# kwea123/ngp_pl

Measured on NVIDIA H100. Metric: train_rays_per_sec, higher is better.
Workload: dtype f16

## Files before the change

ngp_pl_b200/csrc/network.cu:

```cuda
#include "common.cuh"
#include "hashgrid.cuh"
#include "mlp.cuh"
#include "wgmma.cuh"
#include "../../include/ngp_b200.h"
#include <math.h>

extern "C" int ngp_abi_version(void) { return NGP_ABI_VERSION; }

unsigned long long g_ngp_launch_count = 0;
extern "C" unsigned long long ngp_launch_count(void) { return __atomic_load_n(&g_ngp_launch_count, __ATOMIC_RELAXED); }

unsigned long long* g_ngp_trace = nullptr;
__global__ void k_trace_stamp(unsigned long long* buf, int id) { trace_mark(buf, id); }
void ngp_trace_stamp(int id, cudaStream_t st) { k_trace_stamp<<<1, 1, 0, st>>>(g_ngp_trace, id); }
extern "C" int ngp_trace_set(void* buf) {
    g_ngp_trace = (unsigned long long*)buf;
    return 0;
}

extern "C" uint32_t ngp_grid_meta(int n_levels, int log2_hashmap_size, int base_resolution, float per_level_scale,
                                  NgpGridMeta* out) {
    if (!out || n_levels < 1 || n_levels > NGP_MAX_LEVELS || log2_hashmap_size < 3 || log2_hashmap_size > 28 ||
        base_resolution < 1 || !(per_level_scale >= 1.0f))
        return 0;
    const float log2_b = log2f(per_level_scale);
    uint64_t offset = 0;
    out->n_levels = n_levels;
    out->hashed_mask = 0;
    for (int l = 0; l < NGP_MAX_LEVELS; ++l) {
        out->offset[l] = 0; out->res[l] = 0; out->scale[l] = 0.f;
    }
    for (int l = 0; l < n_levels; ++l) {
        const float scale = exp2f((float)l * log2_b) * (float)base_resolution - 1.0f;
        const uint32_t res = (uint32_t)ceilf(scale) + 1u;
        const uint64_t dense = (uint64_t)res * res * res;
        uint64_t entries = (dense + 7u) / 8u * 8u;
        const uint64_t cap = 1ull << log2_hashmap_size;
        if (entries > cap) entries = cap;
        if (dense > entries) out->hashed_mask |= (1u << l);
        out->offset[l] = (uint32_t)offset;
        out->res[l] = res;
        out->scale[l] = scale;
        offset += entries;
        if (offset > 0xffffffffull) return 0;
    }
    for (int l = n_levels; l <= NGP_MAX_LEVELS; ++l) out->offset[l] = (uint32_t)offset;
    return (uint32_t)offset;
}

__global__ void k_cast_params(const float* __restrict__ src, __half* __restrict__ dst, int64_t n) {
    const int64_t i = (blockIdx.x * (int64_t)blockDim.x + threadIdx.x) * 4;
    if (i + 3 < n && ((((uintptr_t)src) & 15) == 0) && ((((uintptr_t)dst) & 7) == 0)) {
        const float4 v = *reinterpret_cast<const float4*>(src + i);
        uint2 o;
        o.x = pack_half2(v.x, v.y);
        o.y = pack_half2(v.z, v.w);
        *reinterpret_cast<uint2*>(dst + i) = o;
    } else {
        for (int64_t k = i; k < n && k < i + 4; ++k) dst[k] = __float2half_rn(src[k]);
    }
}
extern "C" int ngp_cast_params(const float* src, uint16_t* dst_half, int64_t n, void* stream) {
    if (n < 0) return NGP_EINVAL;
    if (n == 0) return 0;
    k_cast_params<<<ngp_div_up((n + 3) / 4, 256), 256, 0, (cudaStream_t)stream>>>(src, (__half*)dst_half, n);
    NGP_CHECK_LAUNCH();
    return 0;
}

#define NGP_SCHED_EAGER 1024
#define NGP_SCHED_GRAPH 1024
__device__ int g_sched[NGP_SCHED_EAGER + NGP_SCHED_GRAPH][2];
static int* sched_slot(cudaStream_t st) {
    static int* bases[64] = {nullptr};
    static unsigned eager_seq[64] = {0}, graph_seq[64] = {0};
    int dev = 0;
    if (cudaGetDevice(&dev) != cudaSuccess || dev < 0 || dev >= 64) return nullptr;
    int* base = __atomic_load_n(&bases[dev], __ATOMIC_ACQUIRE);
    if (!base) {
        void* p = nullptr;
        if (cudaGetSymbolAddress(&p, g_sched) != cudaSuccess) return nullptr;
        base = (int*)p;
        __atomic_store_n(&bases[dev], base, __ATOMIC_RELEASE);
    }
    cudaStreamCaptureStatus cs = cudaStreamCaptureStatusNone;
    if (cudaStreamIsCapturing(st, &cs) != cudaSuccess) return nullptr;
    if (cs != cudaStreamCaptureStatusNone) {
        const unsigned k = __atomic_fetch_add(&graph_seq[dev], 1u, __ATOMIC_RELAXED);
        return base + 2 * (size_t)(NGP_SCHED_EAGER + k % NGP_SCHED_GRAPH);
    }
    return base + 2 * (size_t)(__atomic_fetch_add(&eager_seq[dev], 1u, __ATOMIC_RELAXED) % NGP_SCHED_EAGER);
}
__device__ __forceinline__ void sched_finish(int* sched) {
    if (!sched) return;
    __syncthreads();
    if (threadIdx.x == 0) {
        __threadfence();
        if (atomicAdd(&sched[1], 1) == (int)gridDim.x - 1) {
            sched[0] = 0;
            sched[1] = 0;
            __threadfence();
        }
    }
}

struct SampleIn {
    float x, y, z;
    float dx, dy, dz;
};
__device__ __forceinline__ int64_t sample_count(const NgpSamples& s) {
    if (s.n_dev) {
        const int64_t v = (int64_t)__ldg(s.n_dev);
        return v < s.n ? (v < 0 ? 0 : v) : s.n;
    }
    return s.n;
}

__device__ __forceinline__ int64_t bwd_count(const NgpSamples& s) {
    if (s.live_idx) {
        const int64_t v = (int64_t)__ldg(s.n_live_dev);
        return v < s.n ? (v < 0 ? 0 : v) : s.n;
    }
    return sample_count(s);
}

__device__ __forceinline__ SampleIn load_sample(const NgpSamples& s, int64_t i, bool& valid) {
    SampleIn o;
    if (!valid) {
        o.x = o.y = o.z = 0.f;
        o.dx = 0.f; o.dy = 0.f; o.dz = 1.f;
        return o;
    }
    if (s.ray_idx) {
        const int r = __ldg(s.ray_idx + i);
        if (r < 0) {
            valid = false;
            o.x = o.y = o.z = 0.f;
            o.dx = 0.f; o.dy = 0.f; o.dz = 1.f;
            return o;
        }
        const float t = __ldg(s.ts + i);
        o.dx = __ldg(s.rays_d + 3 * r); o.dy = __ldg(s.rays_d + 3 * r + 1); o.dz = __ldg(s.rays_d + 3 * r + 2);
        o.x = __fmaf_rn(o.dx, t, __ldg(s.rays_o + 3 * r));
        o.y = __fmaf_rn(o.dy, t, __ldg(s.rays_o + 3 * r + 1));
        o.z = __fmaf_rn(o.dz, t, __ldg(s.rays_o + 3 * r + 2));
    } else {
        o.x = __ldg(s.xyzs + 3 * i); o.y = __ldg(s.xyzs + 3 * i + 1); o.z = __ldg(s.xyzs + 3 * i + 2);
        if (s.dirs) {
            o.dx = __ldg(s.dirs + 3 * i); o.dy = __ldg(s.dirs + 3 * i + 1); o.dz = __ldg(s.dirs + 3 * i + 2);
        } else {
            o.dx = 0.f; o.dy = 0.f; o.dz = 1.f;
        }
    }
    return o;
}

__device__ __forceinline__ float sel4(int q, float a, float b, float c, float d) {
    return q == 0 ? a : (q == 1 ? b : (q == 2 ? c : d));
}

__device__ __forceinline__ void to_unit(const NgpNet& net, const SampleIn& s, float& u, float& v, float& w) {
    u = __fdiv_rn(s.x - net.xyz_min[0], net.xyz_max[0] - net.xyz_min[0]);
    v = __fdiv_rn(s.y - net.xyz_min[1], net.xyz_max[1] - net.xyz_min[1]);
    w = __fdiv_rn(s.z - net.xyz_min[2], net.xyz_max[2] - net.xyz_min[2]);
}

template <int MT>
__device__ __forceinline__ void encode_rows(const NgpNet& net, const uint32_t* __restrict__ table,
                                            const float (&u)[MT][2][3], const bool (&valid)[MT][2],
                                            uint32_t (&featA)[MT][2][4], int q) {
#pragma unroll
    for (int mt = 0; mt < MT; ++mt)
#pragma unroll
        for (int h = 0; h < 2; ++h)
#pragma unroll
            for (int j = 0; j < 4; ++j) {
                const int level = 4 * j + q;
                float2 f = make_float2(0.f, 0.f);
                if (valid[mt][h] && level < net.meta.n_levels)
                    f = grid_lookup(table, net.meta, level, u[mt][h][0], u[mt][h][1], u[mt][h][2]);
                featA[mt][j >> 1][2 * (j & 1) + h] = pack_half2(f.x, f.y);
            }
}

__device__ __forceinline__ void sh_rows(const SampleIn& s, int q, uint32_t& lo, uint32_t& hi) {
    const float inv = 1.0f / sqrtf(s.dx * s.dx + s.dy * s.dy + s.dz * s.dz);
    float sh[16];
    sh4(s.dx * inv, s.dy * inv, s.dz * inv, sh);
    lo = pack_half2(sel4(q, sh[0], sh[2], sh[4], sh[6]), sel4(q, sh[1], sh[3], sh[5], sh[7]));
    hi = pack_half2(sel4(q, sh[8], sh[10], sh[12], sh[14]), sel4(q, sh[9], sh[11], sh[13], sh[15]));
}

__device__ __forceinline__ float half_round(float v) { return __half2float(__float2half_rn(v)); }
__device__ __forceinline__ float lo_half(uint32_t u) { return __half2float(__ushort_as_half((unsigned short)(u & 0xffffu))); }
__device__ __forceinline__ float hi_half(uint32_t u) { return __half2float(__ushort_as_half((unsigned short)(u >> 16))); }

#define FWD_MT 1
#define FWD_THREADS 256
#define FWD_MIN_BLOCKS 3
__global__ void __launch_bounds__(FWD_THREADS, FWD_MIN_BLOCKS)
k_ngp_fwd(const NgpNet net, const NgpSamples smp, const int want_rgb, float* __restrict__ sigmas, float* __restrict__ rgbs,
          __half* __restrict__ h_out, uint4* __restrict__ feat_save, int* __restrict__ sched) {
    __shared__ __align__(16) MlpWeightsFwd sw;
    const __half* wd = reinterpret_cast<const __half*>(net.enc_params_h);
    const __half* wr = want_rgb ? reinterpret_cast<const __half*>(net.rgb_params_h) : nullptr;
    load_weights_fwd(sw, wd, wr, threadIdx.x, FWD_THREADS);
    __syncthreads();
    const uint32_t* table = reinterpret_cast<const uint32_t*>(wd + NGP_DENSITY_MLP_PARAMS);

    const int lane = threadIdx.x & 31, g = lane >> 2, q = lane & 3;
    const int64_t n = sample_count(smp);
    const int64_t n_tiles = (n + 16 * FWD_MT - 1) / (16 * FWD_MT);
    const int n_warps = (int)gridDim.x * (FWD_THREADS / 32);
    int grabbed = (int)blockIdx.x * (FWD_THREADS / 32) + (threadIdx.x >> 5);
    if (sched && lane == 0) grabbed = atomicAdd(&sched[0], 1);
    for (;;) {
        const int64_t tile = __shfl_sync(0xffffffffu, grabbed, 0);
        if (tile >= n_tiles) break;
        if (!sched) grabbed += n_warps;
        else if (lane == 0) grabbed = atomicAdd(&sched[0], 1);
        const int64_t base = tile * 16 * FWD_MT;
        SampleIn sm[FWD_MT][2];
        bool valid[FWD_MT][2];
        float u[FWD_MT][2][3];
#pragma unroll
        for (int mt = 0; mt < FWD_MT; ++mt)
#pragma unroll
            for (int h = 0; h < 2; ++h) {
                const int64_t row = base + 16 * mt + g + 8 * h;
                valid[mt][h] = row < n;
                sm[mt][h] = load_sample(smp, row, valid[mt][h]);
                to_unit(net, sm[mt][h], u[mt][h][0], u[mt][h][1], u[mt][h][2]);
            }

        uint32_t featA[FWD_MT][2][4];
        encode_rows<FWD_MT>(net, table, u, valid, featA, q);

        if (feat_save) {
#pragma unroll
            for (int mt = 0; mt < FWD_MT; ++mt)
#pragma unroll
                for (int kt = 0; kt < 2; ++kt)
                    feat_save[((tile * FWD_MT + mt) * 2 + kt) * 32 + lane] =
                        make_uint4(featA[mt][kt][0], featA[mt][kt][1], featA[mt][kt][2], featA[mt][kt][3]);
        }

        uint32_t hidA[FWD_MT][4][4];
        {
            float hidC[FWD_MT][8][4];
            mlp_layer<FWD_MT, 32, 64, LD32>(featA, sw.w1d, hidC, g, q);
            relu_to_frag<FWD_MT, 64>(hidC, hidA);
        }
        uint32_t hA[FWD_MT][1][4];
        {
            float hC[FWD_MT][2][4];
            mlp_layer<FWD_MT, 64, 16, LD64>(hidA, sw.w2d, hC, g, q);
            to_frag<FWD_MT, 16>(hC, hA);
        }
#pragma unroll
        for (int mt = 0; mt < FWD_MT; ++mt)
#pragma unroll
            for (int h = 0; h < 2; ++h) {
                const int64_t row = base + 16 * mt + g + 8 * h;
                if (valid[mt][h]) {
                    if (q == 0) sigmas[row] = expf(lo_half(hA[mt][0][h]));
                    if (h_out) {
                        uint32_t* ho = reinterpret_cast<uint32_t*>(h_out + row * 16);
                        ho[q] = hA[mt][0][h];
                        ho[4 + q] = hA[mt][0][2 + h];
                    }
                }
            }
        if (!want_rgb) continue;

        uint32_t inA[FWD_MT][2][4];
#pragma unroll
        for (int mt = 0; mt < FWD_MT; ++mt) {
#pragma unroll
            for (int h = 0; h < 2; ++h) sh_rows(sm[mt][h], q, inA[mt][0][h], inA[mt][0][2 + h]);
#pragma unroll
            for (int e = 0; e < 4; ++e) inA[mt][1][e] = hA[mt][0][e];
        }
        uint32_t r1A[FWD_MT][4][4];
        {
            float c[FWD_MT][8][4];
            mlp_layer<FWD_MT, 32, 64, LD32>(inA, sw.w1r, c, g, q);
            relu_to_frag<FWD_MT, 64>(c, r1A);
        }
        uint32_t r2A[FWD_MT][4][4];
        {
            float c[FWD_MT][8][4];
            mlp_layer<FWD_MT, 64, 64, LD64>(r1A, sw.w2r, c, g, q);
            relu_to_frag<FWD_MT, 64>(c, r2A);
        }
        float oC[FWD_MT][1][4];
        mlp_layer<FWD_MT, 64, 8, LD64>(r2A, sw.w3r, oC, g, q);
#pragma unroll
        for (int mt = 0; mt < FWD_MT; ++mt)
#pragma unroll
            for (int h = 0; h < 2; ++h) {
                const int64_t row = base + 16 * mt + g + 8 * h;
                if (!valid[mt][h] || q > 1) continue;
                float a = oC[mt][0][2 * h], b = oC[mt][0][2 * h + 1];
                if (net.rgb_act == 1) {
                    a = 1.0f / (1.0f + __expf(-a));
                    b = 1.0f / (1.0f + __expf(-b));
                }
                a = half_round(a);
                b = half_round(b);
                if (q == 0) {
                    rgbs[3 * row] = a;
                    rgbs[3 * row + 1] = b;
                } else {
                    rgbs[3 * row + 2] = a;
                }
            }
    }
    sched_finish(sched);
}

extern "C" int ngp_net_forward(const NgpNet* net, const NgpSamples* smp, int want_rgb, float* sigmas, float* rgbs,
                               uint16_t* h_out, void* feat_save, void* stream) {
    if (!net || !smp || smp->n < 0 || !sigmas || (want_rgb && !rgbs)) return NGP_EINVAL;
    if (net->meta.n_levels < 1 || net->meta.n_levels > NGP_MAX_LEVELS) return NGP_EINVAL;
    if (smp->n == 0) return 0;
    cudaStream_t st = (cudaStream_t)stream;
    const int64_t n_tiles = (smp->n + 16 * FWD_MT - 1) / (16 * FWD_MT);
    const int64_t want = (n_tiles + FWD_THREADS / 32 - 1) / (FWD_THREADS / 32);
    const int64_t cap = (int64_t)ngp_sm_count() * FWD_MIN_BLOCKS;
    const int grid = (int)(want < cap ? want : cap);
    k_ngp_fwd<<<grid, FWD_THREADS, 0, st>>>(*net, *smp, want_rgb, sigmas, rgbs, (__half*)h_out, (uint4*)feat_save,
                                            sched_slot(st));
    NGP_CHECK_LAUNCH();
    NGP_TRACE(3, st);
    return 0;
}

#define B3_WARPS 12
#define B3_ROW_THREADS (B3_WARPS * 32)
#define B3_THREADS (B3_ROW_THREADS + 128)
#define B3_ROWS (B3_WARPS * 16)
struct Bwd3Smem {
    MlpWeightsFwd wf;
    __align__(128) __half feat[B3_ROWS * 32];
    __align__(128) __half hid[B3_ROWS * 64];
    __align__(128) __half rin[B3_ROWS * 32];
    __align__(128) __half r1[B3_ROWS * 64];
    __align__(128) __half r2[B3_ROWS * 64];
    __align__(128) __half dbuf[2][B3_ROWS * 64];
    __align__(8) uint64_t done[2];
    uint64_t staged[5];
    int blk[2];
};

template <int KT>
__device__ __forceinline__ void stage_canon(__half* __restrict__ dst, int C, int row0, const uint32_t (&A)[KT][4], int g, int q) {
    __half* b0 = dst + (row0 >> 3) * (C * 8) + g * 8 + 2 * q;
    __half* b1 = b0 + C * 8;
#pragma unroll
    for (int kt = 0; kt < KT; ++kt) {
        *reinterpret_cast<uint32_t*>(b0 + (2 * kt) * 64) = A[kt][0];
        *reinterpret_cast<uint32_t*>(b1 + (2 * kt) * 64) = A[kt][1];
        *reinterpret_cast<uint32_t*>(b0 + (2 * kt + 1) * 64) = A[kt][2];
        *reinterpret_cast<uint32_t*>(b1 + (2 * kt + 1) * 64) = A[kt][3];
    }
}
template <int KT>
__device__ __forceinline__ void load_canon(const __half* __restrict__ src, int C, int row0, uint32_t (&A)[1][KT][4], int g, int q) {
    const __half* b0 = src + (row0 >> 3) * (C * 8) + g * 8 + 2 * q;
    const __half* b1 = b0 + C * 8;
#pragma unroll
    for (int kt = 0; kt < KT; ++kt) {
        A[0][kt][0] = *reinterpret_cast<const uint32_t*>(b0 + (2 * kt) * 64);
        A[0][kt][1] = *reinterpret_cast<const uint32_t*>(b1 + (2 * kt) * 64);
        A[0][kt][2] = *reinterpret_cast<const uint32_t*>(b0 + (2 * kt + 1) * 64);
        A[0][kt][3] = *reinterpret_cast<const uint32_t*>(b1 + (2 * kt + 1) * 64);
    }
}
template <int N>
__device__ __forceinline__ void wgmma_wgrad(float (&d)[N / 2], const __half* A, const __half* B) {
    const uint32_t lbo_a = 64u * 16u, lbo_b = (uint32_t)N * 16u;
    uint64_t ad = wgmma_smem_desc(A, lbo_a, 128), bd = wgmma_smem_desc(B, lbo_b, 128);
    const uint64_t a_step = (uint64_t)((2u * lbo_a) >> 4), b_step = (uint64_t)((2u * lbo_b) >> 4);
    wgmma_fence_operand(d);
    wgmma_fence();
#pragma unroll
    for (int ks = 0; ks < B3_ROWS / 16; ++ks) {
        wgmma_f16<N>(d, ad, bd);
        ad += a_step;
        bd += b_step;
    }
    wgmma_commit();
    wgmma_wait<0>();
    wgmma_fence_operand(d);
}
template <int N, bool TRANSPOSED>
__device__ __forceinline__ void wgmma_acc_flush(const float (&d)[N / 2], float* dW, int ld, int m0, int q, float inv_scale) {
#pragma unroll
    for (int j = 0; j < N / 8; ++j)
#pragma unroll
        for (int h = 0; h < 2; ++h) {
            const int m = m0 + 8 * h, c = 8 * j + 2 * q;
            const float v0 = d[4 * j + 2 * h] * inv_scale, v1 = d[4 * j + 2 * h + 1] * inv_scale;
            if (TRANSPOSED) {
                asm volatile("red.global.add.f32 [%0], %1;" ::"l"(dW + c * ld + m), "f"(v0) : "memory");
                asm volatile("red.global.add.f32 [%0], %1;" ::"l"(dW + (c + 1) * ld + m), "f"(v1) : "memory");
            } else {
                red_add_f32x2(dW + m * ld + c, v0, v1);
            }
        }
}

template <bool REGATHER>
__global__ void __launch_bounds__(B3_THREADS, 1)
k_ngp_bwd3(const NgpNet net, const NgpSamples smp, const float* __restrict__ dL_dsigmas, const float* __restrict__ dL_drgbs,
           const uint4* __restrict__ feat_save, const float* __restrict__ loss_scale, float* __restrict__ grad_enc,
           float* __restrict__ grad_rgb, uint32_t* __restrict__ dfeat, const int64_t dfeat_stride, int* __restrict__ sched) {
    extern __shared__ __align__(128) unsigned char smem_raw[];
    Bwd3Smem& S = *reinterpret_cast<Bwd3Smem*>(smem_raw);
    const __half* wd = reinterpret_cast<const __half*>(net.enc_params_h);
    const __half* wr = reinterpret_cast<const __half*>(net.rgb_params_h);
    load_weights_fwd(S.wf, wd, wr, threadIdx.x, B3_THREADS);

    const int warp = threadIdx.x >> 5, lane = threadIdx.x & 31, g = lane >> 2, q = lane & 3;
    const bool mma_wg = warp >= B3_WARPS;
    const int64_t n = bwd_count(smp);
    const int32_t* __restrict__ live = smp.live_idx;
    const int64_t n_mtiles = (n + 15) / 16;
    const int64_t n_blks = (n_mtiles + B3_WARPS - 1) / B3_WARPS;
    const float scale = loss_scale ? *loss_scale : 1.0f;
    const float inv_scale = 1.0f / scale;
    const int row0 = 16 * warp;

    if (threadIdx.x == 0) {
        mbar_init(&S.done[0], 4);
        mbar_init(&S.done[1], 4);
#pragma unroll
        for (int l = 0; l < 5; ++l) mbar_init(&S.staged[l], B3_WARPS);
        asm volatile("fence.mbarrier_init.release.cluster;" ::: "memory");
        S.blk[0] = sched ? atomicAdd(&sched[0], 1) : (int)blockIdx.x;
    }
    __syncthreads();
    uint32_t commits[2] = {0u, 0u};

    if (mma_wg) {
        float a3r[8], a2r[32], a1r[16], a2d[8], a1d[16];
#pragma unroll
        for (int i = 0; i < 8; ++i) a3r[i] = a2d[i] = 0.f;
#pragma unroll
        for (int i = 0; i < 16; ++i) a1r[i] = a1d[i] = 0.f;
#pragma unroll
        for (int i = 0; i < 32; ++i) a2r[i] = 0.f;
        auto signal = [&](int b) {
            __syncwarp();
            if (lane == 0) mbar_arrive(&S.done[b]);
        };
        int n_done = 0;
        for (int it = 0;; ++it) {
            const int64_t blk = S.blk[it & 1];
            if (blk >= n_blks) break;
            ++n_done;
            __syncthreads();
            const uint32_t par = (uint32_t)it & 1u;
            mbar_wait(&S.staged[0], par);
            wgmma_wgrad<16>(a3r, S.r2, S.dbuf[0]);   signal(0);
            mbar_wait(&S.staged[1], par);
            wgmma_wgrad<64>(a2r, S.dbuf[1], S.r1);   signal(1);
            mbar_wait(&S.staged[2], par);
            wgmma_wgrad<32>(a1r, S.dbuf[0], S.rin);  signal(0);
            mbar_wait(&S.staged[3], par);
            wgmma_wgrad<16>(a2d, S.hid, S.dbuf[1]);  signal(1);
            mbar_wait(&S.staged[4], par);
            wgmma_wgrad<32>(a1d, S.dbuf[0], S.feat); signal(0);
        }
        sched_finish(sched);
        if (n_done > 0) {
            const int m0 = 16 * (warp - B3_WARPS) + g;
            wgmma_acc_flush<16, true>(a3r, grad_rgb + 2048 + 4096, 64, m0, q, inv_scale);
            wgmma_acc_flush<64, false>(a2r, grad_rgb + 2048, 64, m0, q, inv_scale);
            wgmma_acc_flush<32, false>(a1r, grad_rgb, 32, m0, q, inv_scale);
            wgmma_acc_flush<16, true>(a2d, grad_enc + 2048, 64, m0, q, inv_scale);
            wgmma_acc_flush<32, false>(a1d, grad_enc, 32, m0, q, inv_scale);
        }
        return;
    }

    bool pre_valid[2] = {false, false};
    int64_t pre_src[2] = {0, 0};
    int pre_ridx[2] = {-1, -1};
    float pre_t[2] = {0.f, 0.f};
    float pre_up[2][3] = {{0.f, 0.f, 0.f}, {0.f, 0.f, 0.f}};
    uint32_t pre_feat[2][4] = {{0u, 0u, 0u, 0u}, {0u, 0u, 0u, 0u}};
    auto fetch_hop1 = [&](int64_t nblk) {
#pragma unroll
        for (int h = 0; h < 2; ++h) {
            const int64_t row = (nblk * B3_WARPS + warp) * 16 + g + 8 * h;
            pre_valid[h] = nblk < n_blks && row < n;
            pre_src[h] = pre_valid[h] ? (live ? (int64_t)__ldg(live + row) : row) : 0;
        }
    };
    auto fetch_hop2 = [&](int64_t nblk) {
#pragma unroll
        for (int h = 0; h < 2; ++h) {
            const int64_t sidx = pre_src[h];
            pre_ridx[h] = -1;
            pre_up[h][0] = pre_up[h][1] = pre_up[h][2] = 0.f;
            if (pre_valid[h]) {
                if (smp.ray_idx) {
                    pre_ridx[h] = __ldg(smp.ray_idx + sidx);
                    pre_t[h] = __ldg(smp.ts + sidx);
                }
                if (q == 0) {
                    pre_up[h][0] = __ldg(dL_dsigmas + sidx);
                    pre_up[h][1] = __ldg(dL_drgbs + 3 * sidx);
                    pre_up[h][2] = __ldg(dL_drgbs + 3 * sidx + 1);
                } else if (q == 1) {
                    pre_up[h][1] = __ldg(dL_drgbs + 3 * sidx + 2);
                }
            }
            if constexpr (!REGATHER) {
                const uint32_t* fs = reinterpret_cast<const uint32_t*>(feat_save);
                const int64_t t2 = (sidx >> 4) * 2;
                const int r = (int)(sidx & 15);
                const int64_t w0 = (r & 7) * 4 + q;
                const int sub = r >> 3;
#pragma unroll
                for (int kt = 0; kt < 2; ++kt) {
                    const uint32_t* p = fs + ((t2 + kt) * 32 + w0) * 4 + sub;
                    pre_feat[kt][h] = pre_valid[h] ? __ldg(p) : 0u;
                    pre_feat[kt][2 + h] = pre_valid[h] ? __ldg(p + 2) : 0u;
                }
            }
        }
        (void)nblk;
    };
    fetch_hop1(S.blk[0]);
    fetch_hop2(S.blk[0]);

    auto wait_buf = [&](int b) {
        if (commits[b]) mbar_wait(&S.done[b], (commits[b] - 1u) & 1u);
    };

    for (int it = 0;; ++it) {
        const int64_t blk = S.blk[it & 1];
        if (blk >= n_blks) break;
        if (threadIdx.x == 0) S.blk[(it + 1) & 1] = sched ? atomicAdd(&sched[0], 1) : (int)(blk + gridDim.x);

        const int64_t mtile = blk * B3_WARPS + warp;
        const int64_t base = mtile * 16;
        bool valid[2];
        float up_sig[2], up_c0[2], up_c1[2];
        SampleIn sm[2];
        uint32_t featA[1][2][4];
#pragma unroll
        for (int h = 0; h < 2; ++h) {
            valid[h] = pre_valid[h];
            up_sig[h] = pre_up[h][0]; up_c0[h] = pre_up[h][1]; up_c1[h] = pre_up[h][2];
#pragma unroll
            for (int kt = 0; kt < 2; ++kt) {
                featA[0][kt][h] = pre_feat[kt][h];
                featA[0][kt][2 + h] = pre_feat[kt][2 + h];
            }
            if (valid[h] && pre_ridx[h] >= 0) {
                const int r = pre_ridx[h];
                const float t = pre_t[h];
                sm[h].dx = __ldg(smp.rays_d + 3 * r); sm[h].dy = __ldg(smp.rays_d + 3 * r + 1); sm[h].dz = __ldg(smp.rays_d + 3 * r + 2);
                sm[h].x = __fmaf_rn(sm[h].dx, t, __ldg(smp.rays_o + 3 * r));
                sm[h].y = __fmaf_rn(sm[h].dy, t, __ldg(smp.rays_o + 3 * r + 1));
                sm[h].z = __fmaf_rn(sm[h].dz, t, __ldg(smp.rays_o + 3 * r + 2));
            } else {
                bool v = valid[h];
                sm[h] = load_sample(smp, pre_src[h], v);
                valid[h] = v;
            }
        }
        if constexpr (REGATHER) {
            const uint32_t* table = reinterpret_cast<const uint32_t*>(wd + NGP_DENSITY_MLP_PARAMS);
            const bool v[1][2] = {{valid[0], valid[1]}};
            float u[1][2][3];
#pragma unroll
            for (int h = 0; h < 2; ++h) to_unit(net, sm[h], u[0][h][0], u[0][h][1], u[0][h][2]);
            encode_rows<1>(net, table, u, v, featA, q);
        }
        wait_buf(0);
        __syncthreads();
        const int64_t nblk = S.blk[(it + 1) & 1];
        fetch_hop1(nblk);

        stage_canon<2>(S.feat, 32, row0, featA[0], g, q);
        float h0[2];
        uint32_t hA[1][1][4];
        {
            uint32_t hidA[1][4][4];
            {
                float c[1][8][4];
                mlp_layer<1, 32, 64, LD32>(featA, S.wf.w1d, c, g, q);
                relu_to_frag<1, 64>(c, hidA);
            }
            stage_canon<4>(S.hid, 64, row0, hidA[0], g, q);
            float c[1][2][4];
            mlp_layer<1, 64, 16, LD64>(hidA, S.wf.w2d, c, g, q);
            to_frag<1, 16>(c, hA);
        }
        h0[0] = lo_half(hA[0][0][0]);
        h0[1] = lo_half(hA[0][0][1]);
        uint32_t doutA[1][1][4];
        {
            uint32_t inA[1][2][4];
#pragma unroll
            for (int h = 0; h < 2; ++h) sh_rows(sm[h], q, inA[0][0][h], inA[0][0][2 + h]);
#pragma unroll
            for (int e = 0; e < 4; ++e) inA[0][1][e] = hA[0][0][e];
            stage_canon<2>(S.rin, 32, row0, inA[0], g, q);
            uint32_t r1A[1][4][4];
            {
                float c[1][8][4];
                mlp_layer<1, 32, 64, LD32>(inA, S.wf.w1r, c, g, q);
                relu_to_frag<1, 64>(c, r1A);
            }
            stage_canon<4>(S.r1, 64, row0, r1A[0], g, q);
            uint32_t r2A[1][4][4];
            {
                float c[1][8][4];
                mlp_layer<1, 64, 64, LD64>(r1A, S.wf.w2r, c, g, q);
                relu_to_frag<1, 64>(c, r2A);
            }
            stage_canon<4>(S.r2, 64, row0, r2A[0], g, q);
            float oC[1][1][4];
            mlp_layer<1, 64, 8, LD64>(r2A, S.wf.w3r, oC, g, q);
            doutA[0][0][2] = 0u;
            doutA[0][0][3] = 0u;
#pragma unroll
            for (int h = 0; h < 2; ++h) {
                float d0 = 0.f, d1 = 0.f;
                if (valid[h] && q < 2) {
                    float o0 = oC[0][0][2 * h], o1 = oC[0][0][2 * h + 1];
                    float s0 = 1.f, s1 = 1.f;
                    if (net.rgb_act == 1) {
                        o0 = half_round(1.0f / (1.0f + __expf(-o0)));
                        o1 = half_round(1.0f / (1.0f + __expf(-o1)));
                        s0 = o0 * (1.0f - o0);
                        s1 = o1 * (1.0f - o1);
                    }
                    d0 = up_c0[h] * s0 * scale;
                    d1 = (q == 0) ? up_c1[h] * s1 * scale : 0.f;
                }
                doutA[0][0][h] = pack_half2(d0, d1);
            }
        }

        stage_canon<1>(S.dbuf[0], 16, row0, doutA[0], g, q);
        fence_proxy_async_smem();
        __syncwarp();
        if (lane == 0) mbar_arrive(&S.staged[0]);
        commits[0] += 1u;
        uint32_t dA[1][4][4];
        {
            float c[1][8][4];
            mlp_layer_dgrad<16, 64, LD64>(doutA, S.wf.w3r, c, lane);
            uint32_t act[1][4][4];
            load_canon<4>(S.r2, 64, row0, act, g, q);
            relu_bwd_to_frag<1, 64>(c, act, dA);
        }
        wait_buf(1);
        stage_canon<4>(S.dbuf[1], 64, row0, dA[0], g, q);
        fence_proxy_async_smem();
        __syncwarp();
        if (lane == 0) mbar_arrive(&S.staged[1]);
        commits[1] += 1u;
        {
            float c[1][8][4];
            mlp_layer_dgrad<64, 64, LD64>(dA, S.wf.w2r, c, lane);
            uint32_t act[1][4][4];
            load_canon<4>(S.r1, 64, row0, act, g, q);
            relu_bwd_to_frag<1, 64>(c, act, dA);
        }
        fetch_hop2(nblk);
        wait_buf(0);
        stage_canon<4>(S.dbuf[0], 64, row0, dA[0], g, q);
        fence_proxy_async_smem();
        __syncwarp();
        if (lane == 0) mbar_arrive(&S.staged[2]);
        commits[0] += 1u;
        uint32_t dhA[1][1][4];
        {
            float c[1][2][4];
            mlp_layer_dgrad<64, 16, LD32>(dA, S.wf.w1r + 16, c, lane);
            if (q == 0) {
#pragma unroll
                for (int h = 0; h < 2; ++h)
                    if (valid[h]) c[0][0][2 * h] += up_sig[h] * expf(fminf(fmaxf(h0[h], -15.f), 15.f)) * scale;
            }
            to_frag<1, 16>(c, dhA);
        }
        wait_buf(1);
        stage_canon<1>(S.dbuf[1], 16, row0, dhA[0], g, q);
        fence_proxy_async_smem();
        __syncwarp();
        if (lane == 0) mbar_arrive(&S.staged[3]);
        commits[1] += 1u;
        {
            float c[1][8][4];
            mlp_layer_dgrad<16, 64, LD64>(dhA, S.wf.w2d, c, lane);
            uint32_t act[1][4][4];
            load_canon<4>(S.hid, 64, row0, act, g, q);
            relu_bwd_to_frag<1, 64>(c, act, dA);
        }
        wait_buf(0);
        stage_canon<4>(S.dbuf[0], 64, row0, dA[0], g, q);
        fence_proxy_async_smem();
        __syncwarp();
        if (lane == 0) mbar_arrive(&S.staged[4]);
        commits[0] += 1u;
        {
            float c[1][4][4];
            mlp_layer_dgrad<64, 32, LD32>(dA, S.wf.w1d, c, lane);
#pragma unroll
            for (int h = 0; h < 2; ++h) {
                const int64_t row = base + g + 8 * h;
                if (!valid[h]) continue;
#pragma unroll
                for (int j = 0; j < 4; ++j) {
                    const int level = 4 * j + q;
                    if (level < net.meta.n_levels)
                        dfeat[(int64_t)level * dfeat_stride + row] = pack_half2(c[0][j][2 * h], c[0][j][2 * h + 1]);
                }
            }
        }
    }

    sched_finish(sched);
}

#define SCATTER_THREADS 256
__global__ void __launch_bounds__(SCATTER_THREADS)
k_grid_scatter_merged(const NgpNet net, const NgpSamples smp, const uint32_t* __restrict__ dfeat, const int64_t dfeat_stride,
                      const float* __restrict__ loss_scale, float* __restrict__ grad_table) {
    const int lane = threadIdx.x & 31;
    const int64_t n = bwd_count(smp);
    const float inv_scale = loss_scale ? 1.0f / *loss_scale : 1.0f;
    const int64_t n_pad = (n + 31) & ~(int64_t)31;
    const int n_levels = net.meta.n_levels;

    for (int64_t s = blockIdx.x * (int64_t)SCATTER_THREADS + threadIdx.x; s < n_pad; s += (int64_t)gridDim.x * SCATTER_THREADS) {
        bool valid = s < n;
        const SampleIn sm = load_sample(smp, (valid && smp.live_idx) ? (int64_t)__ldg(smp.live_idx + s) : s, valid);
        float u, v, w;
        to_unit(net, sm, u, v, w);
        const unsigned vmask = __ballot_sync(0xffffffffu, valid);
        uint32_t d_next = valid ? __ldg(dfeat + s) : 0u;
        for (int level = 0; level < n_levels; ++level) {
            const uint32_t d_cur = d_next;
            if (valid && level + 1 < n_levels) d_next = __ldg(dfeat + (int64_t)(level + 1) * dfeat_stride + s);
            const uint32_t res = net.meta.res[level];
            const uint32_t off = net.meta.offset[level];
            const uint32_t entries = net.meta.offset[level + 1] - off;
            const bool hashed = (net.meta.hashed_mask >> level) & 1u;
            const GridCell c = grid_cell(u, v, w, net.meta.scale[level]);
            float2 gr = make_float2(0.f, 0.f);
            if (valid) {
                gr = unpack_half2(d_cur);
                gr.x *= inv_scale;
                gr.y *= inv_scale;
            }
            float acc[16];
            {
                float wk[8];
                grid_corner_weights(c, wk);
#pragma unroll
                for (int k = 0; k < 8; ++k) {
                    acc[2 * k] = wk[k] * gr.x;
                    acc[2 * k + 1] = wk[k] * gr.y;
                }
            }
            const uint32_t px = __shfl_up_sync(0xffffffffu, c.gx, 1), py = __shfl_up_sync(0xffffffffu, c.gy, 1),
                           pz = __shfl_up_sync(0xffffffffu, c.gz, 1);
            const bool pvalid = lane > 0 && ((vmask >> (lane - 1)) & 1u);
            const bool head = lane == 0 || !valid || !pvalid || px != c.gx || py != c.gy || pz != c.gz;
            const unsigned heads = __ballot_sync(0xffffffffu, head);
            if (heads != 0xffffffffu) {
                const unsigned later = lane == 31 ? 0u : (heads >> (lane + 1));
                const int run_end = later ? lane + __ffs(later) - 1 : 31;
                unsigned cont = ~heads;
                int max_run = 1;
                while (cont) {
                    cont &= cont >> 1;
                    ++max_run;
                }
                for (int d = 1; d < max_run; d <<= 1) {
                    const bool take = lane + d <= run_end;
#pragma unroll
                    for (int k = 0; k < 16; ++k) {
                        const float o = __shfl_down_sync(0xffffffffu, acc[k], d);
                        if (take) acc[k] += o;
                    }
                }
            }
            if (valid && head) {
                uint32_t idx[8];
                grid_corner_indices(c, res, entries, hashed, idx);
                const float* lvl = grad_table + 2 * (size_t)off;
                grid_scatter_cell_paired(lvl, idx, acc);
            }
        }
    }
}

extern "C" size_t ngp_net_backward_workspace(int64_t n) {
    if (n < 0) return 0;
    const int64_t n16 = (n + 15) / 16 * 16;
    return (size_t)n16 * NGP_MAX_LEVELS * sizeof(uint32_t);
}

static int check_bwd_args(const NgpNet* net, const NgpSamples* smp, void* workspace, size_t workspace_bytes) {
    if (!net || !smp || smp->n < 0) return NGP_EINVAL;
    if (net->meta.n_levels < 1 || net->meta.n_levels > NGP_MAX_LEVELS) return NGP_EINVAL;
    if (smp->n > 0 && (!workspace || workspace_bytes < ngp_net_backward_workspace(smp->n))) return NGP_EINVAL;
    return 0;
}

extern "C" int ngp_net_backward_mlp(const NgpNet* net, const NgpSamples* smp, const float* dL_dsigmas, const float* dL_drgbs,
                                    const void* feat_save, const float* loss_scale, float* grad_enc, float* grad_rgb,
                                    void* workspace, size_t workspace_bytes, void* stream) {
    int rc = check_bwd_args(net, smp, workspace, workspace_bytes);
    if (rc) return rc;
    if (!dL_dsigmas || !dL_drgbs || !grad_enc || !grad_rgb) return NGP_EINVAL;
    if (smp->live_idx && (!smp->n_live_dev || !feat_save)) return NGP_EINVAL;
    if (smp->n == 0) return 0;
    {
        static unsigned char attr_set[64] = {0};
        int dev = 0;
        NGP_CUDA(cudaGetDevice(&dev));
        if (dev < 0 || dev >= 64 || !__atomic_load_n(&attr_set[dev], __ATOMIC_ACQUIRE)) {
            NGP_CUDA(cudaFuncSetAttribute(k_ngp_bwd3<false>, cudaFuncAttributeMaxDynamicSharedMemorySize, (int)sizeof(Bwd3Smem) + 128));
            NGP_CUDA(cudaFuncSetAttribute(k_ngp_bwd3<true>, cudaFuncAttributeMaxDynamicSharedMemorySize, (int)sizeof(Bwd3Smem) + 128));
            if (dev >= 0 && dev < 64) __atomic_store_n(&attr_set[dev], 1, __ATOMIC_RELEASE);
        }
    }
    const int64_t n_mtiles = (smp->n + 15) / 16;
    const int64_t n_blks = (n_mtiles + B3_WARPS - 1) / B3_WARPS;
    const int grid = (int)(n_blks < (int64_t)ngp_sm_count() ? n_blks : ngp_sm_count());
    auto* kernel = feat_save ? k_ngp_bwd3<false> : k_ngp_bwd3<true>;
    kernel<<<grid, B3_THREADS, sizeof(Bwd3Smem) + 128, (cudaStream_t)stream>>>(
        *net, *smp, dL_dsigmas, dL_drgbs, (const uint4*)feat_save, loss_scale, grad_enc, grad_rgb, (uint32_t*)workspace,
        n_mtiles * 16, sched_slot((cudaStream_t)stream));
    NGP_CHECK_LAUNCH();
    NGP_TRACE(6, (cudaStream_t)stream);
    return 0;
}

extern "C" int ngp_net_backward_scatter(const NgpNet* net, const NgpSamples* smp, const float* loss_scale, float* grad_enc,
                                        void* workspace, size_t workspace_bytes, void* stream) {
    int rc = check_bwd_args(net, smp, workspace, workspace_bytes);
    if (rc) return rc;
    if (!grad_enc || (smp->live_idx && !smp->n_live_dev)) return NGP_EINVAL;
    if (smp->n == 0) return 0;
    const int64_t n_mtiles = (smp->n + 15) / 16;
    int64_t gx = (smp->n + SCATTER_THREADS - 1) / SCATTER_THREADS;
    const int64_t cap = (int64_t)ngp_sm_count() * 8;
    if (gx > cap) gx = cap;
    k_grid_scatter_merged<<<(unsigned)gx, SCATTER_THREADS, 0, (cudaStream_t)stream>>>(
        *net, *smp, (const uint32_t*)workspace, n_mtiles * 16, loss_scale, grad_enc + NGP_DENSITY_MLP_PARAMS);
    NGP_CHECK_LAUNCH();
    NGP_TRACE(7, (cudaStream_t)stream);
    return 0;
}

extern "C" int ngp_net_backward(const NgpNet* net, const NgpSamples* smp, const float* dL_dsigmas, const float* dL_drgbs,
                                const void* feat_save, const float* loss_scale, float* grad_enc, float* grad_rgb,
                                void* workspace, size_t workspace_bytes, void* stream) {
    int rc = ngp_net_backward_mlp(net, smp, dL_dsigmas, dL_drgbs, feat_save, loss_scale, grad_enc, grad_rgb, workspace,
                                  workspace_bytes, stream);
    if (rc) return rc;
    return ngp_net_backward_scatter(net, smp, loss_scale, grad_enc, workspace, workspace_bytes, stream);
}

__global__ void k_grad_amax(const float* __restrict__ dsig, const float* __restrict__ sig, const float* __restrict__ drgb,
                            int64_t n, float* __restrict__ amax) {
    float m = 0.f;
    for (int64_t i = blockIdx.x * (int64_t)blockDim.x + threadIdx.x; i < n; i += (int64_t)gridDim.x * blockDim.x) {
        const float s = fminf(sig[i], 3.2690173e6f);
        m = fmaxf(m, fabsf(dsig[i] * s));
        m = fmaxf(m, fmaxf(fabsf(drgb[3 * i]), fmaxf(fabsf(drgb[3 * i + 1]), fabsf(drgb[3 * i + 2]))));
    }
    m = warp_max(m);
    if ((threadIdx.x & 31) == 0 && m > 0.f && m < INFINITY) atomicMax(reinterpret_cast<int*>(amax), __float_as_int(m));
}
__global__ void k_grad_scale(float* __restrict__ amax, float* __restrict__ scale_out) {
    const float m = *amax;
    float s = 1.0f;
    if (m > 0.f && m < INFINITY) {
        int e;
        frexpf(256.0f / m, &e);
        e = max(-60, min(60, e - 1));
        s = scalbnf(1.0f, e);
    }
    *scale_out = s;
    *amax = 0.f;
}
extern "C" int ngp_grad_scale(const float* dL_dsigmas, const float* sigmas, const float* dL_drgbs, int64_t n,
                              float* scratch, float* scale_out, void* stream) {
    if (n < 0 || !scratch || !scale_out) return NGP_EINVAL;
    cudaStream_t st = (cudaStream_t)stream;
    NGP_CUDA(cudaMemsetAsync(scratch, 0, sizeof(float), st));
    if (n > 0) {
        int grid = ngp_div_up(n, 256);
        if (grid > 4 * ngp_sm_count()) grid = 4 * ngp_sm_count();
        k_grad_amax<<<grid, 256, 0, st>>>(dL_dsigmas, sigmas, dL_drgbs, n, scratch);
        NGP_CHECK_LAUNCH();
    }
    k_grad_scale<<<1, 1, 0, st>>>(scratch, scale_out);
    NGP_CHECK_LAUNCH();
    return 0;
}
```

ngp_pl_b200/csrc/wgmma.cuh:

```cuda
#pragma once
#include <cuda_runtime.h>
#include <stdint.h>

__device__ __forceinline__ uint64_t wgmma_smem_desc(const void* smem, uint32_t lbo_bytes, uint32_t sbo_bytes) {
    const uint32_t a = (uint32_t)__cvta_generic_to_shared(smem);
    uint64_t d = 0;
    d |= (uint64_t)((a >> 4) & 0x3fffu);
    d |= (uint64_t)((lbo_bytes >> 4) & 0x3fffu) << 16;
    d |= (uint64_t)((sbo_bytes >> 4) & 0x3fffu) << 32;
    return d;
}

template <int N>
__device__ __forceinline__ void wgmma_f16(float (&d)[N / 2], uint64_t adesc, uint64_t bdesc);
template <>
__device__ __forceinline__ void wgmma_f16<16>(float (&d)[8], uint64_t adesc, uint64_t bdesc) {
    asm volatile(
        "{\n\t.reg .pred p;\n\tsetp.ne.b32 p, %10, 0;\n\t"
        "wgmma.mma_async.sync.aligned.m64n16k16.f32.f16.f16 {%0,%1,%2,%3,%4,%5,%6,%7}, %8, %9, p, 1, 1, 1, 1;\n}\n"
        : "+f"(d[0]), "+f"(d[1]), "+f"(d[2]), "+f"(d[3]), "+f"(d[4]), "+f"(d[5]), "+f"(d[6]), "+f"(d[7])
        : "l"(adesc), "l"(bdesc), "r"(1)
        : "memory");
}
template <>
__device__ __forceinline__ void wgmma_f16<32>(float (&d)[16], uint64_t adesc, uint64_t bdesc) {
    asm volatile(
        "{\n\t.reg .pred p;\n\tsetp.ne.b32 p, %18, 0;\n\t"
        "wgmma.mma_async.sync.aligned.m64n32k16.f32.f16.f16 {%0,%1,%2,%3,%4,%5,%6,%7,%8,%9,%10,%11,%12,%13,%14,%15}, %16, %17, p, 1, 1, 1, 1;\n}\n"
        : "+f"(d[0]), "+f"(d[1]), "+f"(d[2]), "+f"(d[3]), "+f"(d[4]), "+f"(d[5]), "+f"(d[6]), "+f"(d[7]), "+f"(d[8]), "+f"(d[9]), "+f"(d[10]), "+f"(d[11]), "+f"(d[12]), "+f"(d[13]), "+f"(d[14]), "+f"(d[15])
        : "l"(adesc), "l"(bdesc), "r"(1)
        : "memory");
}
template <>
__device__ __forceinline__ void wgmma_f16<64>(float (&d)[32], uint64_t adesc, uint64_t bdesc) {
    asm volatile(
        "{\n\t.reg .pred p;\n\tsetp.ne.b32 p, %34, 0;\n\t"
        "wgmma.mma_async.sync.aligned.m64n64k16.f32.f16.f16 {%0,%1,%2,%3,%4,%5,%6,%7,%8,%9,%10,%11,%12,%13,%14,%15,%16,%17,%18,%19,%20,%21,%22,%23,%24,%25,%26,%27,%28,%29,%30,%31}, %32, %33, p, 1, 1, 1, 1;\n}\n"
        : "+f"(d[0]), "+f"(d[1]), "+f"(d[2]), "+f"(d[3]), "+f"(d[4]), "+f"(d[5]), "+f"(d[6]), "+f"(d[7]), "+f"(d[8]), "+f"(d[9]), "+f"(d[10]), "+f"(d[11]), "+f"(d[12]), "+f"(d[13]), "+f"(d[14]), "+f"(d[15]), "+f"(d[16]), "+f"(d[17]), "+f"(d[18]), "+f"(d[19]), "+f"(d[20]), "+f"(d[21]), "+f"(d[22]), "+f"(d[23]), "+f"(d[24]), "+f"(d[25]), "+f"(d[26]), "+f"(d[27]), "+f"(d[28]), "+f"(d[29]), "+f"(d[30]), "+f"(d[31])
        : "l"(adesc), "l"(bdesc), "r"(1)
        : "memory");
}

__device__ __forceinline__ void wgmma_fence() { asm volatile("wgmma.fence.sync.aligned;" ::: "memory"); }
__device__ __forceinline__ void wgmma_commit() { asm volatile("wgmma.commit_group.sync.aligned;" ::: "memory"); }
template <int N>
__device__ __forceinline__ void wgmma_wait() { asm volatile("wgmma.wait_group.sync.aligned %0;" ::"n"(N) : "memory"); }
template <int R>
__device__ __forceinline__ void wgmma_fence_operand(float (&d)[R]) {
#pragma unroll
    for (int i = 0; i < R; ++i) asm volatile("" : "+f"(d[i])::"memory");
}
__device__ __forceinline__ void fence_proxy_async_smem() { asm volatile("fence.proxy.async.shared::cta;" ::: "memory"); }

__device__ __forceinline__ void mbar_init(uint64_t* mbar, uint32_t count) {
    asm volatile("mbarrier.init.shared::cta.b64 [%0], %1;" ::"r"((uint32_t)__cvta_generic_to_shared(mbar)), "r"(count) : "memory");
}
__device__ __forceinline__ void mbar_arrive(uint64_t* mbar) {
    asm volatile("mbarrier.arrive.shared::cta.b64 _, [%0];" ::"r"((uint32_t)__cvta_generic_to_shared(mbar)) : "memory");
}
__device__ __forceinline__ void mbar_wait(uint64_t* mbar, uint32_t parity) {
    const uint32_t a = (uint32_t)__cvta_generic_to_shared(mbar);
    const long long t0 = clock64();
    for (;;) {
        uint32_t done;
        asm volatile(
            "{\n\t"
            ".reg .pred p;\n\t"
            "mbarrier.try_wait.parity.shared::cta.b64 p, [%1], %2;\n\t"
            "selp.u32 %0, 1, 0, p;\n\t"
            "}\n"
            : "=r"(done)
            : "r"(a), "r"(parity)
            : "memory");
        if (done) return;
        if (clock64() - t0 > 4000000000ll) asm volatile("trap;");
    }
}
```

Measured before the change: 15.49 million.

## Switch backward MLP layers from per-warp mma.sync to warpgroup wgmma

Replaces the per-warp mma.sync forward-recompute and dgrad layers in the backward kernel with warpgroup-level wgmma that takes its A operand from registers. Weights now live in shared memory in the canonical wgmma layout, loaded with cp.async and made visible to the async proxy with a fence. Transposed B descriptors serve the dgrad products, so no separate transposed weight copy is needed. The aim is to cut instruction-issue and shared-memory fragment-load cost for the small matrices. In exchange, every layer adds a commit and a full wait, which serialises the layers and requires all four warps of each warpgroup to stay in lockstep.

```diff
diff --git a/ngp_pl_b200/csrc/network.cu b/ngp_pl_b200/csrc/network.cu
--- a/ngp_pl_b200/csrc/network.cu
+++ b/ngp_pl_b200/csrc/network.cu
@@ -340,8 +340,49 @@
 #define B3_ROW_THREADS (B3_WARPS * 32)
 #define B3_THREADS (B3_ROW_THREADS + 128)
 #define B3_ROWS (B3_WARPS * 16)
+struct MlpWeightsCanon {
+    __align__(128) __half w1d[64 * 32];
+    __half w2d[16 * 64];
+    __half w1r[64 * 32];
+    __half w2r[64 * 64];
+    __half w3r[16 * 64];
+};
+__device__ __forceinline__ void load_matrix_canon(__half* dst, const __half* __restrict__ src, int rows, int cols, int tid,
+                                                  int nthreads) {
+    const int cpr = cols >> 3;
+    for (int i = tid; i < rows * cpr; i += nthreads) {
+        const int r = i / cpr, c = i - r * cpr;
+        cp_async_16(dst + (r >> 3) * (cols * 8) + c * 64 + (r & 7) * 8, src + r * cols + 8 * c);
+    }
+}
+__device__ __forceinline__ void load_weights_canon(MlpWeightsCanon& s, const __half* __restrict__ wd, const __half* __restrict__ wr,
+                                                   int tid, int nthreads) {
+    load_matrix_canon(s.w1d, wd, 64, 32, tid, nthreads);
+    load_matrix_canon(s.w2d, wd + 2048, 16, 64, tid, nthreads);
+    load_matrix_canon(s.w1r, wr, 64, 32, tid, nthreads);
+    load_matrix_canon(s.w2r, wr + 2048, 64, 64, tid, nthreads);
+    load_matrix_canon(s.w3r, wr + 2048 + 4096, 16, 64, tid, nthreads);
+}
+
+template <int K, int N, int IN, bool DGRAD>
+__device__ __forceinline__ void wg_layer(const uint32_t (&A)[1][K / 16][4], const __half* W, float (&C)[1][N / 8][4]) {
+    constexpr uint32_t along_in = 128, along_out = IN * 16;
+    constexpr uint32_t lbo = DGRAD ? along_out : along_in, sbo = DGRAD ? along_in : along_out;
+    const uint64_t desc = wgmma_smem_desc(W, lbo, sbo);
+    wgmma_fence_operand(C[0]);
+    wgmma_fence();
+#pragma unroll
+    for (int kt = 0; kt < K / 16; ++kt)
+        wgmma_f16_rs<N, DGRAD ? 1 : 0>(C[0], A[0][kt], desc + (uint64_t)kt * ((2u * lbo) >> 4), kt > 0 ? 1 : 0);
+    wgmma_commit();
+    wgmma_wait<0>();
+    wgmma_fence_operand(C[0]);
+#pragma unroll
+    for (int kt = 0; kt < K / 16; ++kt) wgmma_fence_operand(A[0][kt]);
+}
+
 struct Bwd3Smem {
-    MlpWeightsFwd wf;
+    MlpWeightsCanon w;
     __align__(128) __half feat[B3_ROWS * 32];
     __align__(128) __half hid[B3_ROWS * 64];
     __align__(128) __half rin[B3_ROWS * 32];
@@ -420,7 +461,9 @@
     Bwd3Smem& S = *reinterpret_cast<Bwd3Smem*>(smem_raw);
     const __half* wd = reinterpret_cast<const __half*>(net.enc_params_h);
     const __half* wr = reinterpret_cast<const __half*>(net.rgb_params_h);
-    load_weights_fwd(S.wf, wd, wr, threadIdx.x, B3_THREADS);
+    load_weights_canon(S.w, wd, wr, threadIdx.x, B3_THREADS);
+    cp_async_wait_all();
+    fence_proxy_async_smem();
 
     const int warp = threadIdx.x >> 5, lane = threadIdx.x & 31, g = lane >> 2, q = lane & 3;
     const bool mma_wg = warp >= B3_WARPS;
@@ -594,12 +637,12 @@
             uint32_t hidA[1][4][4];
             {
                 float c[1][8][4];
-                mlp_layer<1, 32, 64, LD32>(featA, S.wf.w1d, c, g, q);
+                wg_layer<32, 64, 32, false>(featA, S.w.w1d, c);
                 relu_to_frag<1, 64>(c, hidA);
             }
             stage_canon<4>(S.hid, 64, row0, hidA[0], g, q);
             float c[1][2][4];
-            mlp_layer<1, 64, 16, LD64>(hidA, S.wf.w2d, c, g, q);
+            wg_layer<64, 16, 64, false>(hidA, S.w.w2d, c);
             to_frag<1, 16>(c, hA);
         }
         h0[0] = lo_half(hA[0][0][0]);
@@ -615,19 +658,19 @@
             uint32_t r1A[1][4][4];
             {
                 float c[1][8][4];
-                mlp_layer<1, 32, 64, LD32>(inA, S.wf.w1r, c, g, q);
+                wg_layer<32, 64, 32, false>(inA, S.w.w1r, c);
                 relu_to_frag<1, 64>(c, r1A);
             }
             stage_canon<4>(S.r1, 64, row0, r1A[0], g, q);
             uint32_t r2A[1][4][4];
             {
                 float c[1][8][4];
-                mlp_layer<1, 64, 64, LD64>(r1A, S.wf.w2r, c, g, q);
+                wg_layer<64, 64, 64, false>(r1A, S.w.w2r, c);
                 relu_to_frag<1, 64>(c, r2A);
             }
             stage_canon<4>(S.r2, 64, row0, r2A[0], g, q);
             float oC[1][1][4];
-            mlp_layer<1, 64, 8, LD64>(r2A, S.wf.w3r, oC, g, q);
+            wg_layer<64, 8, 64, false>(r2A, S.w.w3r, oC);
             doutA[0][0][2] = 0u;
             doutA[0][0][3] = 0u;
 #pragma unroll
@@ -657,7 +700,7 @@
         uint32_t dA[1][4][4];
         {
             float c[1][8][4];
-            mlp_layer_dgrad<16, 64, LD64>(doutA, S.wf.w3r, c, lane);
+            wg_layer<16, 64, 64, true>(doutA, S.w.w3r, c);
             uint32_t act[1][4][4];
             load_canon<4>(S.r2, 64, row0, act, g, q);
             relu_bwd_to_frag<1, 64>(c, act, dA);
@@ -670,7 +713,7 @@
         commits[1] += 1u;
         {
             float c[1][8][4];
-            mlp_layer_dgrad<64, 64, LD64>(dA, S.wf.w2r, c, lane);
+            wg_layer<64, 64, 64, true>(dA, S.w.w2r, c);
             uint32_t act[1][4][4];
             load_canon<4>(S.r1, 64, row0, act, g, q);
             relu_bwd_to_frag<1, 64>(c, act, dA);
@@ -685,7 +728,7 @@
         uint32_t dhA[1][1][4];
         {
             float c[1][2][4];
-            mlp_layer_dgrad<64, 16, LD32>(dA, S.wf.w1r + 16, c, lane);
+            wg_layer<64, 16, 32, true>(dA, S.w.w1r + 2 * 64, c);
             if (q == 0) {
 #pragma unroll
                 for (int h = 0; h < 2; ++h)
@@ -701,7 +744,7 @@
         commits[1] += 1u;
         {
             float c[1][8][4];
-            mlp_layer_dgrad<16, 64, LD64>(dhA, S.wf.w2d, c, lane);
+            wg_layer<16, 64, 64, true>(dhA, S.w.w2d, c);
             uint32_t act[1][4][4];
             load_canon<4>(S.hid, 64, row0, act, g, q);
             relu_bwd_to_frag<1, 64>(c, act, dA);
@@ -714,7 +757,7 @@
         commits[0] += 1u;
         {
             float c[1][4][4];
-            mlp_layer_dgrad<64, 32, LD32>(dA, S.wf.w1d, c, lane);
+            wg_layer<64, 32, 32, true>(dA, S.w.w1d, c);
 #pragma unroll
             for (int h = 0; h < 2; ++h) {
                 const int64_t row = base + g + 8 * h;
diff --git a/ngp_pl_b200/csrc/wgmma.cuh b/ngp_pl_b200/csrc/wgmma.cuh
--- a/ngp_pl_b200/csrc/wgmma.cuh
+++ b/ngp_pl_b200/csrc/wgmma.cuh
@@ -41,6 +41,64 @@
         : "memory");
 }
 
+template <int N, int TRANS_B>
+__device__ __forceinline__ void wgmma_f16_rs(float (&d)[N / 8][4], const uint32_t (&a)[4], uint64_t bdesc, int accumulate);
+template <>
+__device__ __forceinline__ void wgmma_f16_rs<8, 0>(float (&d)[1][4], const uint32_t (&a)[4], uint64_t bdesc, int accumulate) {
+    asm volatile(
+        "{\n\t.reg .pred p;\n\tsetp.ne.b32 p, %9, 0;\n\t"
+        "wgmma.mma_async.sync.aligned.m64n8k16.f32.f16.f16 {%0,%1,%2,%3}, {%4,%5,%6,%7}, %8, p, 1, 1, 0;\n}\n"
+        : "+f"(d[0][0]), "+f"(d[0][1]), "+f"(d[0][2]), "+f"(d[0][3])
+        : "r"(a[0]), "r"(a[1]), "r"(a[2]), "r"(a[3]), "l"(bdesc), "r"(accumulate)
+        : "memory");
+}
+#define WGMMA_RS_16(TB)                                                                                                        \
+    template <>                                                                                                                \
+    __device__ __forceinline__ void wgmma_f16_rs<16, TB>(float (&d)[2][4], const uint32_t (&a)[4], uint64_t bdesc,            \
+                                                         int accumulate) {                                                     \
+        asm volatile(                                                                                                          \
+            "{\n\t.reg .pred p;\n\tsetp.ne.b32 p, %13, 0;\n\t"                                                                 \
+            "wgmma.mma_async.sync.aligned.m64n16k16.f32.f16.f16 {%0,%1,%2,%3,%4,%5,%6,%7}, {%8,%9,%10,%11}, %12, p, 1, 1, " #TB \
+            ";\n}\n"                                                                                                           \
+            : "+f"(d[0][0]), "+f"(d[0][1]), "+f"(d[0][2]), "+f"(d[0][3]), "+f"(d[1][0]), "+f"(d[1][1]), "+f"(d[1][2]),         \
+              "+f"(d[1][3])                                                                                                    \
+            : "r"(a[0]), "r"(a[1]), "r"(a[2]), "r"(a[3]), "l"(bdesc), "r"(accumulate)                                          \
+            : "memory");                                                                                                       \
+    }
+WGMMA_RS_16(0)
+WGMMA_RS_16(1)
+#undef WGMMA_RS_16
+template <>
+__device__ __forceinline__ void wgmma_f16_rs<32, 1>(float (&d)[4][4], const uint32_t (&a)[4], uint64_t bdesc, int accumulate) {
+    asm volatile(
+        "{\n\t.reg .pred p;\n\tsetp.ne.b32 p, %21, 0;\n\t"
+        "wgmma.mma_async.sync.aligned.m64n32k16.f32.f16.f16 {%0,%1,%2,%3,%4,%5,%6,%7,%8,%9,%10,%11,%12,%13,%14,%15}, "
+        "{%16,%17,%18,%19}, %20, p, 1, 1, 1;\n}\n"
+        : "+f"(d[0][0]), "+f"(d[0][1]), "+f"(d[0][2]), "+f"(d[0][3]), "+f"(d[1][0]), "+f"(d[1][1]), "+f"(d[1][2]), "+f"(d[1][3]),
+          "+f"(d[2][0]), "+f"(d[2][1]), "+f"(d[2][2]), "+f"(d[2][3]), "+f"(d[3][0]), "+f"(d[3][1]), "+f"(d[3][2]), "+f"(d[3][3])
+        : "r"(a[0]), "r"(a[1]), "r"(a[2]), "r"(a[3]), "l"(bdesc), "r"(accumulate)
+        : "memory");
+}
+#define WGMMA_RS_64(TB)                                                                                                        \
+    template <>                                                                                                                \
+    __device__ __forceinline__ void wgmma_f16_rs<64, TB>(float (&d)[8][4], const uint32_t (&a)[4], uint64_t bdesc,            \
+                                                         int accumulate) {                                                     \
+        asm volatile(                                                                                                          \
+            "{\n\t.reg .pred p;\n\tsetp.ne.b32 p, %37, 0;\n\t"                                                                 \
+            "wgmma.mma_async.sync.aligned.m64n64k16.f32.f16.f16 {%0,%1,%2,%3,%4,%5,%6,%7,%8,%9,%10,%11,%12,%13,%14,%15,%16,"    \
+            "%17,%18,%19,%20,%21,%22,%23,%24,%25,%26,%27,%28,%29,%30,%31}, {%32,%33,%34,%35}, %36, p, 1, 1, " #TB ";\n}\n"      \
+            : "+f"(d[0][0]), "+f"(d[0][1]), "+f"(d[0][2]), "+f"(d[0][3]), "+f"(d[1][0]), "+f"(d[1][1]), "+f"(d[1][2]),         \
+              "+f"(d[1][3]), "+f"(d[2][0]), "+f"(d[2][1]), "+f"(d[2][2]), "+f"(d[2][3]), "+f"(d[3][0]), "+f"(d[3][1]),         \
+              "+f"(d[3][2]), "+f"(d[3][3]), "+f"(d[4][0]), "+f"(d[4][1]), "+f"(d[4][2]), "+f"(d[4][3]), "+f"(d[5][0]),         \
+              "+f"(d[5][1]), "+f"(d[5][2]), "+f"(d[5][3]), "+f"(d[6][0]), "+f"(d[6][1]), "+f"(d[6][2]), "+f"(d[6][3]),         \
+              "+f"(d[7][0]), "+f"(d[7][1]), "+f"(d[7][2]), "+f"(d[7][3])                                                       \
+            : "r"(a[0]), "r"(a[1]), "r"(a[2]), "r"(a[3]), "l"(bdesc), "r"(accumulate)                                          \
+            : "memory");                                                                                                       \
+    }
+WGMMA_RS_64(0)
+WGMMA_RS_64(1)
+#undef WGMMA_RS_64
+
 __device__ __forceinline__ void wgmma_fence() { asm volatile("wgmma.fence.sync.aligned;" ::: "memory"); }
 __device__ __forceinline__ void wgmma_commit() { asm volatile("wgmma.commit_group.sync.aligned;" ::: "memory"); }
 template <int N>
@@ -49,6 +107,15 @@
 __device__ __forceinline__ void wgmma_fence_operand(float (&d)[R]) {
 #pragma unroll
     for (int i = 0; i < R; ++i) asm volatile("" : "+f"(d[i])::"memory");
+}
+template <int J>
+__device__ __forceinline__ void wgmma_fence_operand(float (&d)[J][4]) {
+#pragma unroll
+    for (int j = 0; j < J; ++j) wgmma_fence_operand(d[j]);
+}
+__device__ __forceinline__ void wgmma_fence_operand(const uint32_t (&a)[4]) {
+#pragma unroll
+    for (int i = 0; i < 4; ++i) asm volatile("" ::"r"(a[i]) : "memory");
 }
 __device__ __forceinline__ void fence_proxy_async_smem() { asm volatile("fence.proxy.async.shared::cta;" ::: "memory"); }
 
```

Result: no change. 15.67 million (median of 6 runs) (+1.2%).
